# sdbds/ACE-Step-1.5-for-windows

Hardware: AMD Instinct MI355X
Metric: songs/sec (30 s audio @ 27 DiT steps, CFG 7 + APG, batch 8 in total, DiT + VAE decode) (higher is better)
Workload: dtype bf16; 1 GPU; acestep-5Hz base DiT (24L/2048d, 1.575B params, random init) + Oobleck decoder, 30 s audio (T=750), 27 steps, CFG 7 (2x8 sequences/forward on rank 0), L=769, 8 songs per request over 1 GPU(s); infer_steps=27, batch_per_gpu=8, batch_rank0=8, global_batch=8, parallelism=dp1, tiny=False, sampler_chains_per_gpu=1, batch_dependent_bits=True

## Files before the change

### ace-step-1.5-for-windows_amd/csrc/conv.hip

```cpp
#include <stdio.h>
#include <stdlib.h>

#include "common.h"


namespace ace355 {

namespace {

__device__ __forceinline__ int lds_off(int row, int slot) { return row * 128 + ((slot ^ ((row >> 1) & 7)) << 4); }

__device__ unsigned long long g_conv_probe[8];

typedef unsigned int u32x4 __attribute__((ext_vector_type(4)));
__device__ __forceinline__ u32x4 ld_u32x4(const void* p) {
    return *reinterpret_cast<const __attribute__((address_space(1))) u32x4*>(reinterpret_cast<uintptr_t>(p));
}

__device__ __forceinline__ void conv_glds16_v(const void* vptr, unsigned lds_addr) {
    unsigned keep;
    asm volatile("s_mov_b32 %0, m0\n\ts_mov_b32 m0, %2\n\ts_nop 0\n\tglobal_load_lds_dwordx4 %1, off\n\ts_mov_b32 m0, %0"
                 : "=&s"(keep)
                 : "v"(vptr), "s"(lds_addr)
                 : "memory");
}

constexpr int HALO_MAX = 64;

__device__ __forceinline__ void conv_glds16(unsigned voff, const void* sbase, unsigned lds_addr) {
    unsigned keep;
    asm volatile("s_mov_b32 %0, m0\n\ts_mov_b32 m0, %3\n\ts_nop 0\n\tglobal_load_lds_dwordx4 %1, %2\n\ts_mov_b32 m0, %0"
                 : "=&s"(keep)
                 : "v"(voff), "s"(sbase), "s"(lds_addr)
                 : "memory");
}

__device__ __forceinline__ bf16x8 frag_kperm(const char* base, int row, int q, int h) {
    const uint2 lo = *reinterpret_cast<const uint2*>(base + lds_off(row, 2 * q) + 8 * h);
    const uint2 hi = *reinterpret_cast<const uint2*>(base + lds_off(row, 2 * q + 1) + 8 * h);
    return as_bf16x8(make_uint4(lo.x, lo.y, hi.x, hi.y));
}

template <int BN, int TM, int WS = 0>
__global__ __launch_bounds__(TM * 2, TM / 64) void conv_kernel(ConvArgs a) {
    static_assert(TM == 128 || (TM == 256 && BN == 128), "tile shapes");
    static_assert(WS == 0 || (TM == 256 && BN == 128), "the 32 x 128 wave shape belongs to the fused 8-wave form");
    constexpr int NTHR = TM * 2;
    constexpr int WIN_MAX = TM + HALO_MAX;
    constexpr int MT = WS ? 1 : ((BN == 128) ? 2 : 1);
    constexpr int NT = WS ? 4 : ((BN == 128) ? 2 : 1);
    constexpr int WCH = BN * 8 / NTHR;
    constexpr int FUSE_LDS = (BN == 128 && TM == 128) ? (BN * 128 + 2048) : (WS ? 2048 : 0);
    __shared__ __attribute__((aligned(16))) char smem[WIN_MAX * 128 + 2 * BN * 128 + FUSE_LDS];
    char* As = smem;
    char* Wbase = smem + WIN_MAX * 128;

    const int tid = threadIdx.x, lane = tid & 63, wave = tid >> 6;
    const int lq = lane & 31, half = lane >> 5;
    const int wm = WS ? wave : ((BN == 128) ? (wave >> 1) : wave);
    const int wn = WS ? 0 : ((BN == 128) ? (wave & 1) : 0);
    int bx = blockIdx.x, by = blockIdx.y;
    if (a.ras_tn > 1) {
        const int L = blockIdx.x, tn = a.ras_tn, full = (a.ras_tm >> 3) << 3;
        if (L < full * tn) {
            const int q = L >> 3;
            by = q % tn;
            bx = (q / tn) * 8 + (L & 7);
        } else {
            const int l2 = L - full * tn;
            by = l2 % tn;
            bx = full + l2 / tn;
        }
    }
    const int m0 = bx * TM, n0 = by * BN, b = blockIdx.z;
    const int Cin = a.Cin, taps = a.taps, dil = a.dil;
    const int win_rows = TM + (taps - 1) * dil;
    const int x_row0 = m0 - a.center * dil;
    const bf16_t* xb = a.x + (long)b * a.x_batch_stride;
    const long wrow = (long)taps * Cin;

    f32x16 acc[MT][NT];
#pragma unroll
    for (int i = 0; i < MT; ++i)
#pragma unroll
        for (int j = 0; j < NT; ++j)
#pragma unroll
            for (int r = 0; r < 16; ++r) acc[i][j][r] = 0.f;

    const int sslot = tid & 7;
    constexpr int NWV = NTHR / 64;
    static_assert(WCH * NWV * 8 == BN, "pieces split evenly over the waves");
    unsigned w_voff[WCH];
    int wst[WCH];
#pragma unroll
    for (int i = 0; i < WCH; ++i) {
        const int prow = 8 * (wave + NWV * i) + (lane >> 3);
        const int ls = (lane & 7) ^ ((prow >> 1) & 7);
        w_voff[i] = (unsigned)(((long)min(n0 + prow, a.N - 1) * wrow + ls * 8) * 2);
        wst[i] = lds_off((tid >> 3) + (NTHR / 8) * i, sslot);
    }
    const unsigned wlds0 = (unsigned)(uintptr_t)Wbase + (unsigned)__builtin_amdgcn_readfirstlane(wave) * 1024u;
    auto w_piece = [&](int i, int tap, int ci0, int buf) {
        const bf16_t* sb = a.w + (long)tap * Cin + ci0;
        const unsigned lb = (unsigned)__builtin_amdgcn_readfirstlane((int)(wlds0 + (unsigned)buf * (BN * 128)));
        conv_glds16(w_voff[i], sb, lb + (unsigned)i * (NWV * 1024));
    };
    auto w_issue = [&](int tap, int ci0, int buf) {
#pragma unroll
        for (int i = 0; i < WCH; ++i) w_piece(i, tap, ci0, buf);
    };
    auto w2_piece = [&](int i, int c2, unsigned lbase) {
        const int prow = 8 * (wave + NWV * i) + (lane >> 3);
        const int ls = (lane & 7) ^ ((prow >> 1) & 7);
        conv_glds16((unsigned)((prow * 128 + ls * 8) * 2), a.w2 + c2 * 64, (unsigned)__builtin_amdgcn_readfirstlane((int)lbase) + (unsigned)i * (NWV * 1024));
    };

    constexpr int WLD = (WIN_MAX * 8 + NTHR - 1) / NTHR;
    constexpr bool PREFETCH = true;
    constexpr bool PARPRE = (TM == 128);
    u32x4 wv[WLD];
    const bool snake = a.alpha != nullptr;
    const int wrow_t = tid >> 3;
    const unsigned x_voff = (unsigned)((wrow_t * Cin + sslot * 8) * 2);
    const long xw_f0 = (long)x_row0 * Cin + a.x_shift;
    const long xw_end = a.x_valid ? a.x_valid : (long)a.L_in * Cin;
    const long xw_fb = max(xw_f0, 0L);
    const int xw_neg = (int)((xw_f0 - xw_fb) * 2);
    const uintptr_t xw_bp = reinterpret_cast<uintptr_t>(xb + xw_fb);
    const unsigned xw_lo32 = (unsigned)__builtin_amdgcn_readfirstlane((int)(unsigned)xw_bp);
    const unsigned xw_hi32 = (unsigned)__builtin_amdgcn_readfirstlane((int)(unsigned)(xw_bp >> 32));
    const unsigned xw_nrec = (unsigned)__builtin_amdgcn_readfirstlane((int)max(0L, min((xw_end - xw_fb) * 2, 0x7fffffffL)));
    const __amdgpu_buffer_rsrc_t x_rsrc =
        __builtin_amdgcn_make_buffer_rsrc(reinterpret_cast<void*>(((uintptr_t)xw_hi32 << 32) | xw_lo32), (short)0, (int)xw_nrec, 0x00020000);
    auto win_load = [&](int ci0) {
#pragma unroll
        for (int i = 0; i < WLD; ++i) {
            const int uoff = xw_neg + (i * (NTHR / 8) * Cin + ci0) * 2;
            const auto v = __builtin_amdgcn_raw_buffer_load_b128(x_rsrc, (int)x_voff + min(uoff, 0), max(uoff, 0), 0);
            wv[i] = __builtin_bit_cast(u32x4, v);
        }
    };
    u32x4 spa[2], spb[2];
    auto par_load = [&](int ci0) {
        if (snake) {
#pragma unroll
            for (int q = 0; q < 2; ++q) {
                spa[q] = ld_u32x4(a.alpha + ci0 + sslot * 8 + 4 * q);
                spb[q] = ld_u32x4(a.beta + ci0 + sslot * 8 + 4 * q);
            }
        }
    };
    const int st0 = lds_off(tid >> 3, sslot);
    auto vec_rsrc = [&](const float* p, int n) {
        const uintptr_t u = reinterpret_cast<uintptr_t>(p);
        const unsigned lo = (unsigned)__builtin_amdgcn_readfirstlane((int)(unsigned)u), hi = (unsigned)__builtin_amdgcn_readfirstlane((int)(unsigned)(u >> 32));
        return __builtin_amdgcn_make_buffer_rsrc(reinterpret_cast<void*>(((uintptr_t)hi << 32) | lo), (short)0, p ? n * 4 : 0, 0x00020000);
    };
    const __amdgpu_buffer_rsrc_t sa_rsrc = vec_rsrc(a.alpha, Cin), sb_rsrc = vec_rsrc(a.beta, Cin);
    auto snake_pair = [&](unsigned p, float a0, unsigned b0, float a1, unsigned b1) -> unsigned {
        const float x0 = bf_lo(p), x1 = bf_hi(p);
        const float s0 = __builtin_amdgcn_sinf(a0 * x0), s1 = __builtin_amdgcn_sinf(a1 * x1);
        return pack_bf2(x0 + __uint_as_float(b0) * s0 * s0, x1 + __uint_as_float(b1) * s1 * s1);
    };
    auto rev4 = [&](const u32x4& v, float (&o)[4]) {
#pragma unroll
        for (int e = 0; e < 4; ++e) o[e] = __uint_as_float(v[e]) * 0.15915494309189535f;
    };
    auto win_store = [&](int ci0) {
        if (snake) {
            if constexpr (PARPRE) {
                float ra[2][4];
                rev4(spa[0], ra[0]); rev4(spa[1], ra[1]);
#pragma unroll
                for (int i = 0; i < WLD; ++i)
#pragma unroll
                    for (int e2 = 0; e2 < 4; ++e2)
                        wv[i][e2] = snake_pair(wv[i][e2], ra[e2 >> 1][2 * (e2 & 1)], spb[e2 >> 1][2 * (e2 & 1)],
                                               ra[e2 >> 1][2 * (e2 & 1) + 1], spb[e2 >> 1][2 * (e2 & 1) + 1]);
            } else {
#pragma unroll
                for (int h = 0; h < 2; ++h) {
                    const u32x4 pa = __builtin_bit_cast(u32x4, __builtin_amdgcn_raw_buffer_load_b128(sa_rsrc, sslot * 32, (ci0 + 4 * h) * 4, 0));
                    const u32x4 pb = __builtin_bit_cast(u32x4, __builtin_amdgcn_raw_buffer_load_b128(sb_rsrc, sslot * 32, (ci0 + 4 * h) * 4, 0));
                    float ra[4];
                    rev4(pa, ra);
#pragma unroll
                    for (int i = 0; i < WLD; ++i)
#pragma unroll
                        for (int q = 0; q < 2; ++q)
                            wv[i][2 * h + q] = snake_pair(wv[i][2 * h + q], ra[2 * q], pb[2 * q], ra[2 * q + 1], pb[2 * q + 1]);
                    __builtin_amdgcn_sched_barrier(0);
                }
            }
        }
#pragma unroll
        for (int i = 0; i < WLD; ++i) {
            const int c = tid + i * NTHR;
            if (c < win_rows * 8) *reinterpret_cast<u32x4*>(As + st0 + i * (NTHR / 8) * 128) = wv[i];
        }
    };
    const bool probe = a.clk_probe && blockIdx.x == gridDim.x / 2 && blockIdx.y == 0 && blockIdx.z == 0 && __builtin_amdgcn_readfirstlane(wave) == 0;
    unsigned long long p_t0 = 0, p_w0 = 0, p_stage = 0, p_taps = 0, p_mark = 0;
    if (probe) p_t0 = clock64(), p_w0 = wall_clock64();
    constexpr bool FPIPE = (TM == 128);
    if (PREFETCH) { win_load(0); if (PARPRE) par_load(0); }
    for (int ci0 = 0; ci0 < Cin; ci0 += 64) {
        if (probe) p_mark = clock64();
        if (!PREFETCH) win_load(ci0);
        __syncthreads();
        if (PREFETCH) __builtin_amdgcn_s_waitcnt(0x0F70);
        w_issue(0, ci0, 0);
        win_store(ci0);
        asm volatile("s_waitcnt vmcnt(0)" ::: "memory");
        __syncthreads();
        if (PREFETCH && ci0 + 64 < Cin) { win_load(ci0 + 64); if (PARPRE) par_load(ci0 + 64); }
        if (probe) { const unsigned long long t = clock64(); p_stage += t - p_mark; p_mark = t; }

#pragma unroll 1
        for (int tap = 0; tap < taps; ++tap) {
            const bool more = (tap + 1) < taps;
            if (more) w_issue(tap + 1, ci0, (tap + 1) & 1);
            if constexpr (FUSE_LDS != 0) {
                if (a.w2 && ci0 + 64 >= Cin) {
                    constexpr int PT_OFF = (WS ? 2 : 3) * BN * 128;
                    if constexpr (WS == 0) {
                        const unsigned w2b = (unsigned)(uintptr_t)(Wbase + 2 * BN * 128) + (unsigned)__builtin_amdgcn_readfirstlane(wave) * 1024u;
                        if (tap >= 1 && tap <= WCH) w2_piece(tap - 1, 0, w2b);
                    }
                    if (tap == 5 && __builtin_amdgcn_readfirstlane(wave) < 2) {
                        const float* src = (wave == 0) ? (lane < 32 ? (a.bias ? a.bias : a.alpha2) : a.alpha2)
                                                       : (lane < 32 ? a.beta2 : (a.bias2 ? a.bias2 : a.beta2));
                        conv_glds16_v(src + 4 * (lane & 31), (unsigned)(uintptr_t)(Wbase + PT_OFF) + (unsigned)__builtin_amdgcn_readfirstlane(wave) * 1024u);
                    }
                    if (!more) {
                        const unsigned ring = wlds0 + (unsigned)((tap + 1) & 1) * (BN * 128);
#pragma unroll
                        for (int i = 0; i < WCH; ++i) w2_piece(i, WS ? 0 : 1, ring);
                    }
                }
            }
            const char* Ws = Wbase + (tap & 1) * (BN * 128);
            const int arow = wm * (MT * 32) + tap * dil + lq;
            if constexpr (FPIPE) {
                bf16x8 fa[2][MT], fw[2][NT];
                auto frag = [&](int kk, int sl) {
#pragma unroll
                    for (int i = 0; i < MT; ++i)
                        fa[sl][i] = as_bf16x8(*reinterpret_cast<const uint4*>(As + lds_off(arow + i * 32, kk * 2 + half)));
#pragma unroll
                    for (int j = 0; j < NT; ++j)
                        fw[sl][j] = as_bf16x8(*reinterpret_cast<const uint4*>(Ws + lds_off(wn * (NT * 32) + j * 32 + lq, kk * 2 + half)));
                };
                frag(0, 0);
#pragma unroll
                for (int kk = 0; kk < 4; ++kk) {
                    if (kk < 3) frag(kk + 1, (kk + 1) & 1);
                    __builtin_amdgcn_sched_barrier(0);
#pragma unroll
                    for (int i = 0; i < MT; ++i)
#pragma unroll
                        for (int j = 0; j < NT; ++j) acc[i][j] = mfma32(fw[kk & 1][j], fa[kk & 1][i], acc[i][j]);
                    __builtin_amdgcn_sched_barrier(0);
                }
            } else {
#pragma unroll
                for (int kk = 0; kk < 4; ++kk) {
                    bf16x8 fa[MT], fw[NT];
#pragma unroll
                    for (int i = 0; i < MT; ++i)
                        fa[i] = as_bf16x8(*reinterpret_cast<const uint4*>(As + lds_off(arow + i * 32, kk * 2 + half)));
#pragma unroll
                    for (int j = 0; j < NT; ++j)
                        fw[j] = as_bf16x8(*reinterpret_cast<const uint4*>(Ws + lds_off(wn * (NT * 32) + j * 32 + lq, kk * 2 + half)));
#pragma unroll
                    for (int i = 0; i < MT; ++i)
#pragma unroll
                        for (int j = 0; j < NT; ++j) acc[i][j] = mfma32(fw[j], fa[i], acc[i][j]);
                }
            }
            if (more) {
                asm volatile("s_waitcnt vmcnt(0)" ::: "memory");
                __syncthreads();
            }
        }
        if (probe) p_taps += clock64() - p_mark;
    }
    const bool full = (m0 + TM <= a.M) && (n0 + BN <= a.N) &&
                      ((long)m0 * a.N + n0 + a.y_shift >= 0) && ((long)(m0 + TM - 1) * a.N + n0 + BN - 1 + a.y_shift < a.y_valid);
    const bool wide = BN == 128 && a.out_mode == 0 && full && a.wide_ok;
    const int mw0 = m0 + wm * (MT * 32), nw0 = n0 + wn * (NT * 32);
    const int row_l = lane >> 2, c4 = lane & 3;
    u32x4 bl[NT], bh[NT];
    u32x4 rv[2][MT * 2];
    const bool has_res = (TM == 128 || WS == 1) && a.res != nullptr;
    auto res_load = [&](int j, u32x4 (&r)[MT * 2]) {
        const long rcol = (long)b * a.res_batch_stride + nw0 + j * 32 + c4 * 8 + a.y_shift;
#pragma unroll
        for (int t = 0; t < MT * 2; ++t) r[t] = ld_u32x4(a.res + rcol + (long)(mw0 + t * 16 + row_l) * a.N);
    };
    auto epi_pre = [&](const float* eb) {
#pragma unroll
        for (int j = 0; j < NT; ++j) {
            bl[j] = u32x4{0u, 0u, 0u, 0u};
            bh[j] = u32x4{0u, 0u, 0u, 0u};
        }
        if (eb && WS == 0) {
#pragma unroll
            for (int j = 0; j < NT; ++j) {
                bl[j] = ld_u32x4(eb + nw0 + j * 32 + c4 * 8);
                bh[j] = ld_u32x4(eb + nw0 + j * 32 + c4 * 8 + 4);
            }
        }
        if (has_res) res_load(0, rv[0]);
    };
    bool epi_pre_done = false;
    const float* epi_bias = a.bias;
    bool bias_in_lds = false;
    if constexpr (WS == 1) {
        if (a.w2) {
            epi_bias = a.bias2;
            bias_in_lds = a.bias2 != nullptr;
            const float b7s = a.bias ? 1.f : 0.f;
            const char* W2c0 = Wbase + (taps & 1) * (BN * 128);
            const char* W2c1 = Wbase + ((taps + 1) & 1) * (BN * 128);
            const char* Pt = Wbase + 2 * BN * 128;
            __syncthreads();
            {
                const unsigned ring = wlds0 + (unsigned)(taps & 1 ? 0 : 1) * (BN * 128);
#pragma unroll
                for (int i = 0; i < WCH; ++i) w2_piece(i, 1, ring);
            }
            uint2 sp[NT][4];
#pragma unroll
            for (int j = 0; j < NT; ++j)
#pragma unroll
                for (int g = 0; g < 4; ++g) {
                    const int c = j * 32 + 8 * g + 4 * half;
                    const u32x4 b4 = *reinterpret_cast<const u32x4*>(Pt + c * 4);
                    const u32x4 e4 = *reinterpret_cast<const u32x4*>(Pt + 512 + c * 4);
                    const u32x4 i4 = *reinterpret_cast<const u32x4*>(Pt + 1024 + c * 4);
                    float t[4];
#pragma unroll
                    for (int e = 0; e < 4; ++e) {
                        const float v = acc[0][j][4 * g + e] + b7s * __uint_as_float(b4[e]);
                        const float sn = __sinf(__uint_as_float(e4[e]) * v);
                        t[e] = v + __uint_as_float(i4[e]) * sn * sn;
                    }
                    sp[j][g] = make_uint2(pack_bf2(t[0], t[1]), pack_bf2(t[2], t[3]));
                    __builtin_amdgcn_sched_barrier(0);
                }
#pragma unroll
            for (int j = 0; j < NT; ++j)
#pragma unroll
                for (int r = 0; r < 16; ++r) acc[0][j][r] = 0.f;
            asm volatile("s_waitcnt vmcnt(0)" ::: "memory");
            __syncthreads();
#pragma unroll
            for (int kg = 0; kg < 8; ++kg) {
                const char* Wp = (kg >> 2) ? W2c1 : W2c0;
                const uint2 s0 = sp[kg >> 1][2 * (kg & 1)], s1 = sp[kg >> 1][2 * (kg & 1) + 1];
                const bf16x8 fb = as_bf16x8(make_uint4(s0.x, s0.y, s1.x, s1.y));
                bf16x8 fw[NT];
#pragma unroll
                for (int j = 0; j < NT; ++j) fw[j] = frag_kperm(Wp, j * 32 + lq, kg & 3, half);
#pragma unroll
                for (int j = 0; j < NT; ++j) acc[0][j] = mfma32(fw[j], fb, acc[0][j]);
            }
        }
    }
    if constexpr (BN == 128 && TM == 128) {
        if (a.w2) {
            epi_bias = a.bias2;
            const float* b7p = a.bias ? a.bias : a.alpha2;
            const float b7s = a.bias ? 1.f : 0.f;
            __syncthreads();
            char* A2 = smem;
            const char* W2c0 = Wbase + 2 * BN * 128;
            const char* W2c1 = Wbase + (taps & 1) * (BN * 128);
            const char* Pt = Wbase + 3 * BN * 128;
#pragma unroll
            for (int j = 0; j < NT; ++j) {
                u32x4 b4[4], e4[4], i4[4];
#pragma unroll
                for (int g = 0; g < 4; ++g) {
                    const int c = n0 + wn * (NT * 32) + j * 32 + 8 * g + 4 * half;
                    b4[g] = *reinterpret_cast<const u32x4*>(Pt + c * 4);
                    e4[g] = *reinterpret_cast<const u32x4*>(Pt + 512 + c * 4);
                    i4[g] = *reinterpret_cast<const u32x4*>(Pt + 1024 + c * 4);
                }
#pragma unroll
                for (int i = 0; i < MT; ++i)
#pragma unroll
                    for (int g = 0; g < 4; ++g) {
                        float t[4];
#pragma unroll
                        for (int e = 0; e < 4; ++e) {
                            const float v = acc[i][j][4 * g + e] + b7s * __uint_as_float(b4[g][e]);
                            const float sn = __sinf(__uint_as_float(e4[g][e]) * v);
                            t[e] = v + __uint_as_float(i4[g][e]) * sn * sn;
                        }
                        const int row = wm * (MT * 32) + i * 32 + lq;
                        uint2 pk = make_uint2(pack_bf2(t[0], t[1]), pack_bf2(t[2], t[3]));
                        *reinterpret_cast<uint2*>(A2 + wn * 16384 + lds_off(row, j * 4 + g) + 8 * half) = pk;
                    }
            }
#pragma unroll
            for (int i = 0; i < MT; ++i)
#pragma unroll
                for (int j = 0; j < NT; ++j)
#pragma unroll
                    for (int r = 0; r < 16; ++r) acc[i][j][r] = 0.f;
            asm volatile("s_waitcnt vmcnt(0)" ::: "memory");
            __syncthreads();
            if (wide) { epi_pre(a.bias2); epi_pre_done = true; }
            {
                bf16x8 fa[2][MT], fw[2][NT];
                auto frag2 = [&](int k8, int sl) {
                    const char* Ap = A2 + (k8 >> 2) * 16384;
                    const char* Wp = (k8 >> 2) ? W2c1 : W2c0;
                    const int kk = k8 & 3;
#pragma unroll
                    for (int i = 0; i < MT; ++i) fa[sl][i] = frag_kperm(Ap, wm * (MT * 32) + i * 32 + lq, kk, half);
#pragma unroll
                    for (int j = 0; j < NT; ++j) fw[sl][j] = frag_kperm(Wp, wn * (NT * 32) + j * 32 + lq, kk, half);
                };
                frag2(0, 0);
#pragma unroll
                for (int k8 = 0; k8 < 8; ++k8) {
                    if (k8 < 7) frag2(k8 + 1, (k8 + 1) & 1);
                    __builtin_amdgcn_sched_barrier(0);
#pragma unroll
                    for (int i = 0; i < MT; ++i)
#pragma unroll
                        for (int j = 0; j < NT; ++j) acc[i][j] = mfma32(fw[k8 & 1][j], fa[k8 & 1][i], acc[i][j]);
                    __builtin_amdgcn_sched_barrier(0);
                }
            }
        }
    }
    const unsigned long long p_e0 = probe ? clock64() : 0ull;
    auto probe_done = [&]() {
        if (!probe) return;
        __builtin_amdgcn_s_waitcnt(0x0F70);
        const unsigned long long t = clock64();
        g_conv_probe[0] = t - p_t0, g_conv_probe[1] = p_stage, g_conv_probe[2] = p_taps, g_conv_probe[3] = t - p_e0;
        g_conv_probe[4] = wall_clock64() - p_w0, g_conv_probe[5] = (unsigned long long)(Cin / 64);
    };

    if (wide) {
        if (!epi_pre_done) epi_pre(epi_bias);
        __syncthreads();
        char* stg = smem + wave * (MT * 32 * 128);
#pragma unroll
        for (int j = 0; j < NT; ++j) {
#pragma unroll
            for (int i = 0; i < MT; ++i)
#pragma unroll
                for (int g = 0; g < 4; ++g) {
                    float4 v;
                    v.x = acc[i][j][4 * g + 0]; v.y = acc[i][j][4 * g + 1]; v.z = acc[i][j][4 * g + 2]; v.w = acc[i][j][4 * g + 3];
                    const int row = i * 32 + lq, slot = 2 * g + half;
                    *reinterpret_cast<float4*>(stg + row * 128 + ((slot ^ (row & 7)) << 4)) = v;
                }
            if (has_res && j + 1 < NT) res_load(j + 1, rv[(j + 1) & 1]);
            u32x4 oa[2], ob[2];
            if (a.osnake_a) {
#pragma unroll
                for (int q = 0; q < 2; ++q) {
                    oa[q] = ld_u32x4(a.osnake_a + nw0 + j * 32 + c4 * 8 + 4 * q);
                    ob[q] = ld_u32x4(a.osnake_b + nw0 + j * 32 + c4 * 8 + 4 * q);
                }
            }
            const long col = (long)b * a.y_batch_stride + nw0 + j * 32 + c4 * 8 + a.y_shift;
            if constexpr (WS == 1) {
                if (bias_in_lds) {
                    const char* pb = Wbase + 2 * BN * 128 + 1536 + (nw0 + j * 32 + c4 * 8) * 4;
                    bl[j] = *reinterpret_cast<const u32x4*>(pb);
                    bh[j] = *reinterpret_cast<const u32x4*>(pb + 16);
                } else if (epi_bias) {
                    bl[j] = ld_u32x4(epi_bias + nw0 + j * 32 + c4 * 8);
                    bh[j] = ld_u32x4(epi_bias + nw0 + j * 32 + c4 * 8 + 4);
                }
            }
            const float bias[8] = {__uint_as_float(bl[j][0]), __uint_as_float(bl[j][1]), __uint_as_float(bl[j][2]), __uint_as_float(bl[j][3]),
                                   __uint_as_float(bh[j][0]), __uint_as_float(bh[j][1]), __uint_as_float(bh[j][2]), __uint_as_float(bh[j][3])};
#pragma unroll
            for (int t = 0; t < MT * 2; ++t) {
                const int row = t * 16 + row_l;
                const float4 lo = *reinterpret_cast<const float4*>(stg + row * 128 + (((2 * c4) ^ (row & 7)) << 4));
                const float4 hi = *reinterpret_cast<const float4*>(stg + row * 128 + (((2 * c4 + 1) ^ (row & 7)) << 4));
                float v[8] = {lo.x + bias[0], lo.y + bias[1], lo.z + bias[2], lo.w + bias[3],
                              hi.x + bias[4], hi.y + bias[5], hi.z + bias[6], hi.w + bias[7]};
                if (has_res) {
                    const u32x4 r = rv[j & 1][t];
#pragma unroll
                    for (int e2 = 0; e2 < 4; ++e2) { v[2 * e2] += bf_lo(r[e2]); v[2 * e2 + 1] += bf_hi(r[e2]); }
                }
                if (a.osnake_a) {
#pragma unroll
                    for (int e = 0; e < 8; ++e) {
                        const float sn = __sinf(__uint_as_float(oa[e >> 2][e & 3]) * v[e]);
                        v[e] = v[e] + __uint_as_float(ob[e >> 2][e & 3]) * sn * sn;
                    }
                }
                u32x4 pk = {pack_bf2(v[0], v[1]), pack_bf2(v[2], v[3]), pack_bf2(v[4], v[5]), pack_bf2(v[6], v[7])};
                *reinterpret_cast<u32x4*>(reinterpret_cast<bf16_t*>(a.y) + col + (long)(mw0 + row) * a.N) = pk;
            }
        }
        probe_done();
        return;
    }
#pragma unroll
    for (int i = 0; i < MT; ++i) {
        const int m = mw0 + i * 32 + lq;
        if (m >= a.M) continue;
#pragma unroll
        for (int j = 0; j < NT; ++j)
#pragma unroll
            for (int r = 0; r < 16; ++r) {
                const int n = nw0 + j * 32 + 8 * (r >> 2) + 4 * half + (r & 3);
                if (n >= a.N) continue;
                float v = acc[i][j][r] + (epi_bias ? epi_bias[n] : 0.f);
                if (a.out_mode == 0) {
                    const long flat = (long)m * a.N + n + a.y_shift;
                    if (flat < 0 || flat >= a.y_valid) continue;
                    if (a.res) v += bf2f(a.res[(long)b * a.res_batch_stride + flat]);
                    if (a.osnake_a) {
                        const float sn = __sinf(a.osnake_a[n] * v);
                        v = v + a.osnake_b[n] * sn * sn;
                    }
                    reinterpret_cast<bf16_t*>(a.y)[(long)b * a.y_batch_stride + flat] = f2bf(v);
                } else {
                    if (n < a.n_real) {
                        if (a.ncl_ld == 0) reinterpret_cast<float*>(a.y)[(long)b * a.y_batch_stride + (long)n * a.M + m] = v;
                        else if (m >= a.ncl_m_lo && m < a.ncl_m_hi)
                            reinterpret_cast<float*>(a.y)[(long)b * a.y_batch_stride + (long)n * a.ncl_ld + a.ncl_off + (m - a.ncl_m_lo)] = v;
                    }
                }
            }
    }
}

__global__ void ncl_to_nlc_kernel(const float* __restrict__ z, bf16_t* __restrict__ out, int C, int T, long total) {
    const long i = (long)blockIdx.x * blockDim.x + threadIdx.x;
    if (i >= total) return;
    const int c = (int)(i % C);
    const long bt = i / C;
    const int t = (int)(bt % T);
    const long b = bt / T;
    out[i] = f2bf(z[(b * C + c) * T + t]);
}

}

int launch_conv(const ConvArgs& a, hipStream_t s) {
    ACE_CHECK(a.Cin % 64 == 0, "conv: Cin must be a multiple of 64");
    ACE_CHECK(a.taps >= 1 && (a.taps - 1) * a.dil <= HALO_MAX && a.dil >= 1, "conv: window too large");
    ACE_CHECK(a.B > 0 && a.M > 0 && a.N > 0, "conv: empty problem");
    ACE_CHECK((long)a.N * a.taps * a.Cin * 2 < (1L << 32) && (reinterpret_cast<uintptr_t>(a.w) & 15) == 0,
              "conv: the weight tensor must be 16-byte aligned and smaller than 4 GB (32-bit DMA offsets)");
    ACE_CHECK(a.x_valid ? (a.x_shift % 8 == 0 && a.x_valid % 8 == 0) : a.x_shift == 0, "conv: x_shift / x_valid must be multiples of 8 (and x_shift needs x_valid)");
    ACE_CHECK(!a.w2 || (a.Cin == 128 && a.N == 128 && a.taps == 7 && !a.x_valid && a.out_mode == 0 && a.alpha2 && a.beta2 &&
                        (reinterpret_cast<uintptr_t>(a.alpha2) & 15) == 0 && (reinterpret_cast<uintptr_t>(a.beta2) & 15) == 0 &&
                        (reinterpret_cast<uintptr_t>(a.bias) & 15) == 0 && (reinterpret_cast<uintptr_t>(a.w2) & 15) == 0),
              "conv: the fused k = 1 stage needs Cin = N = 128, a plain conv and 16-byte aligned vectors");
    ACE_CHECK(!a.osnake_a == !a.osnake_b && (!a.osnake_a || a.out_mode == 0), "conv: the producer-side Snake needs both parameter vectors and the bf16 output");
    ConvArgs aw = a;
    {
        auto al16 = [](const void* p) { return (reinterpret_cast<uintptr_t>(p) & 15) == 0; };
        aw.wide_ok = a.out_mode == 0 && al16(a.y) && al16(a.res) && al16(a.bias) && al16(a.bias2) && al16(a.osnake_a) && al16(a.osnake_b) &&
                     (a.N % 8) == 0 && (a.y_shift % 8) == 0 &&
                     (a.y_batch_stride % 8) == 0 && (a.res_batch_stride % 8) == 0;
    }
    static int tm_env = -1, clk_env = -1, ras_env = -1;
    if (ras_env < 0) {
        const char* e = getenv("ACE355_CONV_RAS");
        ras_env = e ? atoi(e) : 1;
    }
    if (clk_env < 0) {
        const char* e = getenv("ACE355_CONV_CLK");
        clk_env = e ? atoi(e) : 0;
    }
    aw.clk_probe = clk_env;
    if (tm_env < 0) {
        const char* e = getenv("ACE355_CONV_TM");
        tm_env = e ? atoi(e) : 0;
    }
    if (a.N >= 128 || a.N % 128 == 0) {
        const long wgs128 = (long)((a.M + 127) / 128) * ((a.N + 127) / 128) * a.B;
        const bool tall_k = a.Cin >= 128 && a.taps >= 3 && wgs128 >= 1400;
        const bool tall_t = a.taps == 2 && a.Cin >= 128 && !a.alpha && !a.x_valid && wgs128 >= 1500;
        const bool tall = !a.w2 && !a.res && (tm_env ? tm_env == 256 : (tall_k || tall_t));
        const int tm_rows = tall ? 256 : 128;
        dim3 grid((a.M + tm_rows - 1) / tm_rows, (a.N + 127) / 128, a.B);
        aw.ras_tm = aw.ras_tn = 0;
        if (ras_env && grid.y > 1 && (long)grid.x * grid.y < (1L << 31)) {
            aw.ras_tm = (int)grid.x, aw.ras_tn = (int)grid.y;
            grid = dim3(grid.x * grid.y, 1, a.B);
        }
        static int f8_env = -2;
        if (f8_env == -2) {
            const char* e = getenv("ACE355_CONV_F8");
            f8_env = e ? atoi(e) : -1;
        }
        const bool f8 = a.w2 && (f8_env >= 0 ? f8_env != 0 : wgs128 >= 1400);
        if (f8) {
            dim3 g8((a.M + 255) / 256, 1, a.B);
            aw.ras_tm = aw.ras_tn = 0;
            hipLaunchKernelGGL((conv_kernel<128, 256, 1>), g8, dim3(512), 0, s, aw);
        } else
        if (tall) hipLaunchKernelGGL((conv_kernel<128, 256>), grid, dim3(512), 0, s, aw);
        else hipLaunchKernelGGL((conv_kernel<128, 128>), grid, dim3(256), 0, s, aw);
    } else {
        aw.ras_tm = aw.ras_tn = 0;
        dim3 grid((a.M + 127) / 128, (a.N + 31) / 32, a.B);
        hipLaunchKernelGGL((conv_kernel<32, 128>), grid, dim3(256), 0, s, aw);
    }
    ACE_LAUNCH_CHECK();
    if (aw.clk_probe) {
        ACE_HIP(hipStreamSynchronize(s));
        unsigned long long h[8];
        ACE_HIP(hipMemcpyFromSymbol(h, HIP_SYMBOL(g_conv_probe), sizeof(h)));
        fprintf(stderr, "[conv clk] Cin=%d N=%d taps=%d dil=%d M=%d: total %llu cyc = stage %llu + taps %llu + epilogue %llu (+%llu other), wall %.2f us, %llu chunks\n",
                a.Cin, a.N, a.taps, a.dil, a.M, h[0], h[1], h[2], h[3], h[0] - h[1] - h[2] - h[3], h[4] / 100.0, h[5]);
    }
    return 0;
}

int launch_ncl_to_nlc(const float* z, bf16_t* out, int B, int C, int T, hipStream_t s) {
    const long total = (long)B * C * T;
    hipLaunchKernelGGL(ncl_to_nlc_kernel, dim3((unsigned)((total + 255) / 256)), dim3(256), 0, s, z, out, C, T, total);
    ACE_LAUNCH_CHECK();
    return 0;
}

}
```

### ace-step-1.5-for-windows_amd/csrc/vae.hip

```cpp
#include <math.h>
#include <string.h>

#include <algorithm>
#include <map>
#include <string>
#include <vector>

#include "encoder.h"

using namespace ace355;

namespace {

struct ConvW {
    bf16_t* w = nullptr;
    float* bias = nullptr;
    int N = 0, taps = 0, Cin = 0;
};
struct SnakeP {
    float* ea = nullptr;
    float* ib = nullptr;
};
struct ResUnitW {
    SnakeP s1, s2;
// ... 395 lines not shown
    h->finalized = false;
    return ACE355_OK;
}

int ace355_vae_finalize(ace355_vae* h) {
    ACE_CHECK(h, "vae_finalize: null handle");
    const ace355_vae_config& c = h->cfg;
    const int nb = c.num_blocks;
    int cm[ACE355_MAX_BLOCKS + 1];
    cm[0] = 1;
    for (int i = 0; i < nb; ++i) cm[i + 1] = c.channel_multiples[i];
    int rc;
    const int C0 = c.decoder_channels * cm[nb];
    if ((rc = build_conv(h, "decoder.conv1", C0, c.decoder_input_channels, 7, true, &h->conv1))) return rc;
    h->blocks.assign(nb, BlockW());
    for (int i = 0; i < nb; ++i) {
        BlockW& B = h->blocks[i];
        B.cin = c.decoder_channels * cm[nb - i];
        B.cout = c.decoder_channels * cm[nb - i - 1];
        B.stride = c.upsampling_ratios[i];
        B.pad = (B.stride + 1) / 2;
        ACE_CHECK(B.cin % 64 == 0 && B.cout % 64 == 0, "vae_finalize: block channels must be multiples of 64");
        const std::string p = "decoder.block." + std::to_string(i);
        if ((rc = build_snake(h, p + ".snake1", B.cin, &B.s1))) return rc;
        if ((rc = build_convt(h, p + ".conv_t1", B.cin, B.cout, B.stride, &B.ct))) return rc;
        const int dils[3] = {1, 3, 9};
        for (int j = 0; j < 3; ++j) {
            ResUnitW& R = B.ru[j];
            R.dil = dils[j];
            const std::string r = p + ".res_unit" + std::to_string(j + 1);
            if ((rc = build_snake(h, r + ".snake1", B.cout, &R.s1))) return rc;
            if ((rc = build_conv(h, r + ".conv1", B.cout, B.cout, 7, true, &R.c1))) return rc;
            if ((rc = build_snake(h, r + ".snake2", B.cout, &R.s2))) return rc;
            if ((rc = build_conv(h, r + ".conv2", B.cout, B.cout, 1, true, &R.c2))) return rc;
        }
    }
    if ((rc = build_snake(h, "decoder.snake1", c.decoder_channels, &h->s_out))) return rc;
    if ((rc = build_conv(h, "decoder.conv2", c.audio_channels, c.decoder_channels, 7, false, &h->conv2))) return rc;
    h->has_encoder = false;
    for (auto& kv : h->raw) if (kv.first.rfind("encoder.", 0) == 0) { h->has_encoder = true; break; }
    if (h->has_encoder) {
        const int EH = 2 * c.decoder_input_channels;
        ACE_CHECK(EH % 64 == 0, "vae_finalize: encoder width must be a multiple of 64");
        if ((rc = build_conv_im2col(h, "encoder.conv1", EH, c.audio_channels, 7, &h->e_conv1))) return rc;
        h->e_blocks.assign(nb, EncBlockW());
        for (int i = 0; i < nb; ++i) {
            EncBlockW& B = h->e_blocks[i];
            B.cin = EH * cm[i];
            B.cout = EH * cm[i + 1];
            B.stride = c.upsampling_ratios[nb - 1 - i];
            B.pad = (B.stride + 1) / 2;
            ACE_CHECK(B.cin % 64 == 0 && B.cout % 64 == 0, "vae_finalize: encoder block channels must be multiples of 64");
            const std::string p = "encoder.block." + std::to_string(i);
            const int dils[3] = {1, 3, 9};
            for (int j = 0; j < 3; ++j)
                if ((rc = build_res_unit(h, p + ".res_unit" + std::to_string(j + 1), B.cin, dils[j], &B.ru[j]))) return rc;
            if ((rc = build_snake_tiled(h, p + ".snake1", B.cin, B.stride, &B.s1))) return rc;
            if ((rc = build_conv_strided(h, p + ".conv1", B.cout, B.cin, B.stride, &B.cd))) return rc;
        }
        if ((rc = build_snake(h, "encoder.snake1", EH * cm[nb], &h->e_s_out))) return rc;
        if ((rc = build_conv(h, "encoder.conv2", EH, EH * cm[nb], 3, true, &h->e_conv2))) return rc;
    }
    ACE_HIP(hipDeviceSynchronize());
    for (auto& kv : h->raw) {
        const std::string& k = kv.first;
        const bool keep = k.size() > 5 && k.compare(k.size() - 5, 5, ".bias") == 0;
        if (!keep && kv.second.p) { hipFree(kv.second.p); kv.second.p = nullptr; }
    }
    if (!h->scratch) ACE_HIP(hipMalloc((void**)&h->scratch, 1024));
    h->finalized = true;
    return ACE355_OK;
}

int ace355_vae_hop(const ace355_vae* h) { return h ? h->hop : 0; }

static int episnake_on() {
    static int on = -1;
    if (on < 0) {
        const char* e = getenv("ACE355_VAE_EPISNAKE");
        on = e ? atoi(e) : 1;
    }
    return on;
}
static bool unit_fused(int C) {
    static int fuse = -1;
    if (fuse < 0) {
        const char* e = getenv("ACE355_CONV_FUSE_RU");
        fuse = e ? atoi(e) : 1;
    }
    return fuse && C == 128;
}

static void stage_push(std::vector<ace355_vae_stage_info>& v, int kind, int block, int unit, int channels, int flags, int src, int res,
                       int dil, long rows) {
    ace355_vae_stage_info si;
    si.kind = kind; si.block = block; si.unit = unit; si.channels = channels; si.flags = flags; si.src = src; si.res = res;
    si.dilation = dil; si.rows = rows;
    v.push_back(si);
}
static void stage_push_unit(std::vector<ace355_vae_stage_info>& v, int block, int unit, int C, int dil, long rows, bool epi, bool out_snake) {
    const int in = (int)v.size() - 1;
    const int osn = out_snake ? ACE355_VAE_FLAG_OUT_SNAKE : 0;
    if (unit_fused(C)) {
        stage_push(v, ACE355_VAE_STAGE_UNIT, block, unit, C, ACE355_VAE_FLAG_FUSED | ACE355_VAE_FLAG_IN_SNAKE | osn, in, in, dil, rows);
        return;
    }
    stage_push(v, ACE355_VAE_STAGE_UNIT_K7, block, unit, C, ACE355_VAE_FLAG_IN_SNAKE | (epi ? ACE355_VAE_FLAG_OUT_SNAKE : 0), in, -1, dil, rows);
    stage_push(v, ACE355_VAE_STAGE_UNIT_K1, block, unit, C, (epi ? 0 : ACE355_VAE_FLAG_IN_SNAKE) | osn, in + 1, in, 1, rows);
}
static int stage_list(const ace355_vae* h, int enc, long T, std::vector<ace355_vae_stage_info>& v) {
    v.clear();
    const ace355_vae_config& c = h->cfg;
    if (!enc) {
        const bool epi = episnake_on() != 0 && !h->blocks.empty();
        stage_push(v, ACE355_VAE_STAGE_INPUT, -1, -1, c.decoder_input_channels, 0, -1, -1, 1, T);
        stage_push(v, ACE355_VAE_STAGE_CONV_IN, -1, -1, h->conv1.N, epi ? ACE355_VAE_FLAG_OUT_SNAKE : 0, 0, -1, 1, T);
        long L = T;
        for (size_t bi = 0; bi < h->blocks.size(); ++bi) {
            const BlockW& Bk = h->blocks[bi];
            L = (L - 1) * Bk.stride - 2 * Bk.pad + 2 * Bk.stride;
            stage_push(v, ACE355_VAE_STAGE_CONVT, (int)bi, -1, Bk.cout, epi ? 0 : ACE355_VAE_FLAG_IN_SNAKE, (int)v.size() - 1, -1, 1, L);
            for (int j = 0; j < 3; ++j) stage_push_unit(v, (int)bi, j, Bk.cout, Bk.ru[j].dil, L, epi, epi && j == 2);
        }
        return 0;
    }
    const bool epi = episnake_on() != 0;
    const int EH = 2 * c.decoder_input_channels;
    stage_push(v, ACE355_VAE_STAGE_INPUT, -1, -1, 64, 0, -1, -1, 1, T);
    stage_push(v, ACE355_VAE_STAGE_CONV_IN, -1, -1, EH, 0, 0, -1, 1, T);
    long L = T;
    for (size_t bi = 0; bi < h->e_blocks.size(); ++bi) {
        const EncBlockW& Bk = h->e_blocks[bi];
        for (int j = 0; j < 3; ++j) stage_push_unit(v, (int)bi, j, Bk.cin, Bk.ru[j].dil, L, epi, epi && j == 2);
        L = (L + 2 * Bk.pad - 2 * Bk.stride) / Bk.stride + 1;
        ACE_CHECK(L > 0, "vae stages: audio shorter than one latent frame");
        stage_push(v, ACE355_VAE_STAGE_DOWN, (int)bi, -1, Bk.cout,
                   (epi ? 0 : ACE355_VAE_FLAG_IN_SNAKE) | (epi && bi + 1 == h->e_blocks.size() ? ACE355_VAE_FLAG_OUT_SNAKE : 0), (int)v.size() - 1,
                   -1, 1, L);
    }
    stage_push(v, ACE355_VAE_STAGE_HEAD, -1, -1, EH,
               ACE355_VAE_FLAG_F32_NCL | ((!epi || h->e_blocks.empty()) ? ACE355_VAE_FLAG_IN_SNAKE : 0), (int)v.size() - 1, -1, 1, L);
    return 0;
}
static int tap_stage(ace355_vae* h, int enc, int kind, const void* p, int B, hipStream_t s) {
    if (h->tap_stages.empty()) return 0;
    const int k = h->tap_next++;
    ACE_CHECK(k < (int)h->tap_stages.size() && h->tap_stages[k].kind == kind, "vae tap: the stage list and the launch sequence disagree");
    auto it = h->taps[enc].find(k);
    if (it == h->taps[enc].end()) return 0;
    const ace355_vae_stage_info& si = h->tap_stages[k];
    const size_t bytes = (size_t)B * si.rows * si.channels * ((si.flags & ACE355_VAE_FLAG_F32_NCL) ? 4 : 2);
    ACE_CHECK(bytes <= it->second.second, "vae tap: the destination is smaller than the stage");
    ACE_HIP(hipMemcpyAsync(it->second.first, p, bytes, hipMemcpyDeviceToDevice, s));
    return 0;
}
static int tap_begin(ace355_vae* h, int enc, long T, bool single_window) {
    h->tap_stages.clear();
    h->tap_next = 0;
    if (h->taps[enc].empty()) return 0;
    if (!single_window) {
        set_error("vae tap: the call splits into several windows under the activation budget; a tap needs one whole-sequence window");
        return ACE355_ERR_STATE;
    }
    int rc = stage_list(h, enc, T, h->tap_stages);
    if (rc) { h->tap_stages.clear(); return rc; }
    ACE_CHECK(h->taps[enc].rbegin()->first < (int)h->tap_stages.size(), "vae tap: no such stage");
    return 0;
}
static int tap_end(ace355_vae* h) {
    const bool ok = h->tap_stages.empty() || h->tap_next == (int)h->tap_stages.size();
    h->tap_stages.clear();
    ACE_CHECK(ok, "vae tap: the stage list and the launch sequence disagree");
    return 0;
}

static int run_res_unit(ace355_vae* h, const ResUnitW& R, bf16_t*& state, bf16_t*& tmp, int B, long L, int C, hipStream_t s,
                        int enc, const SnakeP* out_snake = nullptr) {
    if (unit_fused(C)) {
        ConvArgs f{};
        f.x = state; f.x_batch_stride = L * C; f.L_in = (int)L; f.Cin = C;
        f.w = R.c1.w; f.bias = R.c1.bias; f.alpha = R.s1.ea; f.beta = R.s1.ib;
        f.w2 = R.c2.w; f.bias2 = R.c2.bias; f.alpha2 = R.s2.ea; f.beta2 = R.s2.ib;
        f.res = state; f.res_batch_stride = L * C;
        f.y = tmp; f.y_batch_stride = L * C;
        f.B = B; f.M = (int)L; f.N = C; f.taps = 7; f.dil = R.dil; f.center = 3;
        f.y_shift = 0; f.y_valid = L * C; f.out_mode = 0;
        if (out_snake) f.osnake_a = out_snake->ea, f.osnake_b = out_snake->ib;
        const int rcf = run_conv(h, f, s);
        if (rcf) return rcf;
        std::swap(state, tmp);
        return tap_stage(h, enc, ACE355_VAE_STAGE_UNIT, state, B, s);
    }
    ConvArgs a{};
    a.x = state; a.x_batch_stride = L * C; a.L_in = (int)L; a.Cin = C;
    a.w = R.c1.w; a.bias = R.c1.bias; a.alpha = R.s1.ea; a.beta = R.s1.ib;
    a.y = tmp; a.y_batch_stride = L * C;
    a.B = B; a.M = (int)L; a.N = C; a.taps = 7; a.dil = R.dil; a.center = 3;
    a.y_shift = 0; a.y_valid = L * C; a.out_mode = 0;
    const bool epi = episnake_on() != 0;
    if (epi) a.osnake_a = R.s2.ea, a.osnake_b = R.s2.ib;
    int rc = run_conv(h, a, s);
    if (rc) return rc;
    if ((rc = tap_stage(h, enc, ACE355_VAE_STAGE_UNIT_K7, tmp, B, s))) return rc;
    a = ConvArgs{};
    a.x = tmp; a.x_batch_stride = L * C; a.L_in = (int)L; a.Cin = C;
    a.w = R.c2.w; a.bias = R.c2.bias;
    if (!epi) a.alpha = R.s2.ea, a.beta = R.s2.ib;
    if (out_snake) a.osnake_a = out_snake->ea, a.osnake_b = out_snake->ib;
    a.res = state; a.res_batch_stride = L * C;
    a.y = state; a.y_batch_stride = L * C;
    a.B = B; a.M = (int)L; a.N = C; a.taps = 1; a.dil = 1; a.center = 0;
    a.y_shift = 0; a.y_valid = L * C; a.out_mode = 0;
    if ((rc = run_conv(h, a, s))) return rc;
    return tap_stage(h, enc, ACE355_VAE_STAGE_UNIT_K1, state, B, s);
}

static size_t decode_elems(const ace355_vae* h, long frames) {
    size_t need = (size_t)frames * h->conv1.N;
    long L = frames;
    for (const BlockW& Bk : h->blocks) {
        L = (L - 1) * Bk.stride - 2 * Bk.pad + 2 * Bk.stride;
        need = std::max(need, (size_t)L * Bk.cout);
    }
    return need;
}
static size_t decode_bytes(const ace355_vae* h, int nb, long frames) { return 3 * (decode_elems(h, frames) * (size_t)nb * 2 + 256); }

static int decode_receptive_frames(const ace355_vae* h) {
    double rf = 3.0, rate = 1.0;
    for (const BlockW& Bk : h->blocks) {
        rf += 1.0 / rate;
        rate *= Bk.stride;
        rf += 3.0 * (1 + 3 + 9) / rate;
    }
    rf += 3.0 / rate;
    return (int)ceil(rf);
}

static int decode_window(ace355_vae* h, int b0, int nb, int T, int ws, int we, int cs, int ce, float* wav_out_dev, hipStream_t s) {
    const ace355_vae_config& c = h->cfg;
    const int Tw = we - ws;
    bf16_t *cur = h->buf[0], *nxt = h->buf[1], *tmp = h->buf[2];
    long L = Tw;
    int rc;
    ConvArgs a{};
    a.x = h->zin + ((size_t)b0 * T + ws) * c.decoder_input_channels; a.x_batch_stride = (long)T * c.decoder_input_channels; a.L_in = Tw;
    a.Cin = c.decoder_input_channels;
    a.w = h->conv1.w; a.bias = h->conv1.bias;
    a.y = cur; a.y_batch_stride = (long)Tw * h->conv1.N;
    a.B = nb; a.M = Tw; a.N = h->conv1.N; a.taps = 7; a.dil = 1; a.center = 3;
    a.y_shift = 0; a.y_valid = (long)Tw * h->conv1.N; a.out_mode = 0;
    const bool epi = episnake_on() != 0 && !h->blocks.empty();
    if (epi) a.osnake_a = h->blocks[0].s1.ea, a.osnake_b = h->blocks[0].s1.ib;
    if ((rc = run_conv(h, a, s))) return rc;
    if ((rc = tap_stage(h, 0, ACE355_VAE_STAGE_CONV_IN, cur, nb, s))) return rc;

    for (size_t bi = 0; bi < h->blocks.size(); ++bi) {
        const BlockW& Bk = h->blocks[bi];
        const SnakeP* next_snake = !epi ? nullptr : (bi + 1 < h->blocks.size() ? &h->blocks[bi + 1].s1 : &h->s_out);
        const long Lout = (L - 1) * Bk.stride - 2 * Bk.pad + 2 * Bk.stride;
        a = ConvArgs{};
// ... 304 lines not shown
```

Before: 17.50 songs/s.

## Extend fused residual-unit conv kernel to 256-channel decoder stages

Generalizes the fused k=7 conv + Snake + k=1 conv residual-unit kernel from 128 channels to 256 channels by adding a 256x256 tile, 8-wave variant. The k=1 weight chunks are streamed through the double-buffered LDS ring with extra barriers, and the parameter and bias vectors are laid out by BN. Decoder residual units at C=256 now use this single kernel instead of separate conv launches, which removes an intermediate activation round-trip through global memory. The trade-offs are a larger LDS footprint and lower occupancy (launch bounds of 2), plus extra synchronization inside the epilogue.

```diff
diff --git a/ace-step-1.5-for-windows_amd/csrc/conv.hip b/ace-step-1.5-for-windows_amd/csrc/conv.hip
--- a/ace-step-1.5-for-windows_amd/csrc/conv.hip
+++ b/ace-step-1.5-for-windows_amd/csrc/conv.hip
@@ -42,15 +42,15 @@
 }
 
 template <int BN, int TM, int WS = 0>
-__global__ __launch_bounds__(TM * 2, TM / 64) void conv_kernel(ConvArgs a) {
-    static_assert(TM == 128 || (TM == 256 && BN == 128), "tile shapes");
-    static_assert(WS == 0 || (TM == 256 && BN == 128), "the 32 x 128 wave shape belongs to the fused 8-wave form");
+__global__ __launch_bounds__(TM * 2, (WS && BN == 256) ? 2 : TM / 64) void conv_kernel(ConvArgs a) {
+    static_assert(TM == 128 || (TM == 256 && (BN == 128 || (BN == 256 && WS == 1))), "tile shapes");
+    static_assert(WS == 0 || (TM == 256 && BN >= 128), "the 32 x BN wave shape belongs to the fused 8-wave forms");
     constexpr int NTHR = TM * 2;
     constexpr int WIN_MAX = TM + HALO_MAX;
     constexpr int MT = WS ? 1 : ((BN == 128) ? 2 : 1);
-    constexpr int NT = WS ? 4 : ((BN == 128) ? 2 : 1);
+    constexpr int NT = WS ? BN / 32 : ((BN == 128) ? 2 : 1);
     constexpr int WCH = BN * 8 / NTHR;
-    constexpr int FUSE_LDS = (BN == 128 && TM == 128) ? (BN * 128 + 2048) : (WS ? 2048 : 0);
+    constexpr int FUSE_LDS = (BN == 128 && TM == 128) ? (BN * 128 + 2048) : (WS ? BN * 16 : 0);
     __shared__ __attribute__((aligned(16))) char smem[WIN_MAX * 128 + 2 * BN * 128 + FUSE_LDS];
     char* As = smem;
     char* Wbase = smem + WIN_MAX * 128;
@@ -112,7 +112,7 @@
     auto w2_piece = [&](int i, int c2, unsigned lbase) {
         const int prow = 8 * (wave + NWV * i) + (lane >> 3);
         const int ls = (lane & 7) ^ ((prow >> 1) & 7);
-        conv_glds16((unsigned)((prow * 128 + ls * 8) * 2), a.w2 + c2 * 64, (unsigned)__builtin_amdgcn_readfirstlane((int)lbase) + (unsigned)i * (NWV * 1024));
+        conv_glds16((unsigned)((prow * BN + ls * 8) * 2), a.w2 + c2 * 64, (unsigned)__builtin_amdgcn_readfirstlane((int)lbase) + (unsigned)i * (NWV * 1024));
     };
 
     constexpr int WLD = (WIN_MAX * 8 + NTHR - 1) / NTHR;
@@ -227,10 +227,11 @@
                         const unsigned w2b = (unsigned)(uintptr_t)(Wbase + 2 * BN * 128) + (unsigned)__builtin_amdgcn_readfirstlane(wave) * 1024u;
                         if (tap >= 1 && tap <= WCH) w2_piece(tap - 1, 0, w2b);
                     }
-                    if (tap == 5 && __builtin_amdgcn_readfirstlane(wave) < 2) {
-                        const float* src = (wave == 0) ? (lane < 32 ? (a.bias ? a.bias : a.alpha2) : a.alpha2)
-                                                       : (lane < 32 ? a.beta2 : (a.bias2 ? a.bias2 : a.beta2));
-                        conv_glds16_v(src + 4 * (lane & 31), (unsigned)(uintptr_t)(Wbase + PT_OFF) + (unsigned)__builtin_amdgcn_readfirstlane(wave) * 1024u);
+                    if (tap == 5 && __builtin_amdgcn_readfirstlane(wave) < BN / 64) {
+                        constexpr int LPV = BN / 4;
+                        const int vec = (wave * 64 + lane) / LPV;
+                        const float* src = vec == 0 ? (a.bias ? a.bias : a.alpha2) : vec == 1 ? a.alpha2 : vec == 2 ? a.beta2 : (a.bias2 ? a.bias2 : a.beta2);
+                        conv_glds16_v(src + 4 * ((wave * 64 + lane) % LPV), (unsigned)(uintptr_t)(Wbase + PT_OFF) + (unsigned)__builtin_amdgcn_readfirstlane(wave) * 1024u);
                     }
                     if (!more) {
                         const unsigned ring = wlds0 + (unsigned)((tap + 1) & 1) * (BN * 128);
@@ -287,7 +288,7 @@
     }
     const bool full = (m0 + TM <= a.M) && (n0 + BN <= a.N) &&
                       ((long)m0 * a.N + n0 + a.y_shift >= 0) && ((long)(m0 + TM - 1) * a.N + n0 + BN - 1 + a.y_shift < a.y_valid);
-    const bool wide = BN == 128 && a.out_mode == 0 && full && a.wide_ok;
+    const bool wide = BN >= 128 && a.out_mode == 0 && full && a.wide_ok;
     const int mw0 = m0 + wm * (MT * 32), nw0 = n0 + wn * (NT * 32);
     const int row_l = lane >> 2, c4 = lane & 3;
     u32x4 bl[NT], bh[NT];
@@ -321,8 +322,7 @@
             epi_bias = a.bias2;
             bias_in_lds = a.bias2 != nullptr;
             const float b7s = a.bias ? 1.f : 0.f;
-            const char* W2c0 = Wbase + (taps & 1) * (BN * 128);
-            const char* W2c1 = Wbase + ((taps + 1) & 1) * (BN * 128);
+            constexpr int NC2 = BN / 64;
             const char* Pt = Wbase + 2 * BN * 128;
             __syncthreads();
             {
@@ -337,8 +337,8 @@
                 for (int g = 0; g < 4; ++g) {
                     const int c = j * 32 + 8 * g + 4 * half;
                     const u32x4 b4 = *reinterpret_cast<const u32x4*>(Pt + c * 4);
-                    const u32x4 e4 = *reinterpret_cast<const u32x4*>(Pt + 512 + c * 4);
-                    const u32x4 i4 = *reinterpret_cast<const u32x4*>(Pt + 1024 + c * 4);
+                    const u32x4 e4 = *reinterpret_cast<const u32x4*>(Pt + BN * 4 + c * 4);
+                    const u32x4 i4 = *reinterpret_cast<const u32x4*>(Pt + BN * 8 + c * 4);
                     float t[4];
 #pragma unroll
                     for (int e = 0; e < 4; ++e) {
@@ -356,15 +356,30 @@
             asm volatile("s_waitcnt vmcnt(0)" ::: "memory");
             __syncthreads();
 #pragma unroll
-            for (int kg = 0; kg < 8; ++kg) {
-                const char* Wp = (kg >> 2) ? W2c1 : W2c0;
-                const uint2 s0 = sp[kg >> 1][2 * (kg & 1)], s1 = sp[kg >> 1][2 * (kg & 1) + 1];
-                const bf16x8 fb = as_bf16x8(make_uint4(s0.x, s0.y, s1.x, s1.y));
-                bf16x8 fw[NT];
-#pragma unroll
-                for (int j = 0; j < NT; ++j) fw[j] = frag_kperm(Wp, j * 32 + lq, kg & 3, half);
-#pragma unroll
-                for (int j = 0; j < NT; ++j) acc[0][j] = mfma32(fw[j], fb, acc[0][j]);
+            for (int c2 = 0; c2 < NC2; ++c2) {
+                const char* Wp = Wbase + ((taps + c2) & 1) * (BN * 128);
+#pragma unroll
+                for (int k4 = 0; k4 < 4; ++k4) {
+                    const int kg = 4 * c2 + k4;
+                    const uint2 s0 = sp[kg >> 1][2 * (kg & 1)], s1 = sp[kg >> 1][2 * (kg & 1) + 1];
+                    const bf16x8 fb = as_bf16x8(make_uint4(s0.x, s0.y, s1.x, s1.y));
+                    bf16x8 fw[NT];
+#pragma unroll
+                    for (int j = 0; j < NT; ++j) fw[j] = frag_kperm(Wp, j * 32 + lq, k4, half);
+#pragma unroll
+                    for (int j = 0; j < NT; ++j) acc[0][j] = mfma32(fw[j], fb, acc[0][j]);
+                }
+                if constexpr (NC2 > 2) {
+                    if (c2 + 1 < NC2) {
+                        asm volatile("s_waitcnt vmcnt(0)" ::: "memory");
+                        __syncthreads();
+                        if (c2 + 2 < NC2) {
+                            const unsigned ring = wlds0 + (unsigned)((taps + c2) & 1) * (BN * 128);
+#pragma unroll
+                            for (int i = 0; i < WCH; ++i) w2_piece(i, c2 + 2, ring);
+                        }
+                    }
+                }
             }
         }
     }
@@ -474,7 +489,7 @@
             const long col = (long)b * a.y_batch_stride + nw0 + j * 32 + c4 * 8 + a.y_shift;
             if constexpr (WS == 1) {
                 if (bias_in_lds) {
-                    const char* pb = Wbase + 2 * BN * 128 + 1536 + (nw0 + j * 32 + c4 * 8) * 4;
+                    const char* pb = Wbase + 2 * BN * 128 + BN * 12 + (nw0 + j * 32 + c4 * 8) * 4;
                     bl[j] = *reinterpret_cast<const u32x4*>(pb);
                     bh[j] = *reinterpret_cast<const u32x4*>(pb + 16);
                 } else if (epi_bias) {
@@ -560,10 +575,11 @@
     ACE_CHECK((long)a.N * a.taps * a.Cin * 2 < (1L << 32) && (reinterpret_cast<uintptr_t>(a.w) & 15) == 0,
               "conv: the weight tensor must be 16-byte aligned and smaller than 4 GB (32-bit DMA offsets)");
     ACE_CHECK(a.x_valid ? (a.x_shift % 8 == 0 && a.x_valid % 8 == 0) : a.x_shift == 0, "conv: x_shift / x_valid must be multiples of 8 (and x_shift needs x_valid)");
-    ACE_CHECK(!a.w2 || (a.Cin == 128 && a.N == 128 && a.taps == 7 && !a.x_valid && a.out_mode == 0 && a.alpha2 && a.beta2 &&
+    ACE_CHECK(!a.w2 || ((a.Cin == 128 || a.Cin == 256) && a.N == a.Cin && a.taps == 7 && !a.x_valid && a.out_mode == 0 && a.alpha2 && a.beta2 &&
                         (reinterpret_cast<uintptr_t>(a.alpha2) & 15) == 0 && (reinterpret_cast<uintptr_t>(a.beta2) & 15) == 0 &&
-                        (reinterpret_cast<uintptr_t>(a.bias) & 15) == 0 && (reinterpret_cast<uintptr_t>(a.w2) & 15) == 0),
-              "conv: the fused k = 1 stage needs Cin = N = 128, a plain conv and 16-byte aligned vectors");
+                        (reinterpret_cast<uintptr_t>(a.bias) & 15) == 0 && (reinterpret_cast<uintptr_t>(a.bias2) & 15) == 0 &&
+                        (reinterpret_cast<uintptr_t>(a.w2) & 15) == 0),
+              "conv: the fused k = 1 stage needs Cin = N = 128 or 256, a plain conv and 16-byte aligned vectors");
     ACE_CHECK(!a.osnake_a == !a.osnake_b && (!a.osnake_a || a.out_mode == 0), "conv: the producer-side Snake needs both parameter vectors and the bf16 output");
     ConvArgs aw = a;
     {
@@ -604,6 +620,11 @@
             f8_env = e ? atoi(e) : -1;
         }
         const bool f8 = a.w2 && (f8_env >= 0 ? f8_env != 0 : wgs128 >= 1400);
+        if (a.w2 && a.N == 256) {
+            dim3 g8((a.M + 255) / 256, 1, a.B);
+            aw.ras_tm = aw.ras_tn = 0;
+            hipLaunchKernelGGL((conv_kernel<256, 256, 1>), g8, dim3(512), 0, s, aw);
+        } else
         if (f8) {
             dim3 g8((a.M + 255) / 256, 1, a.B);
             aw.ras_tm = aw.ras_tn = 0;
diff --git a/ace-step-1.5-for-windows_amd/csrc/vae.hip b/ace-step-1.5-for-windows_amd/csrc/vae.hip
--- a/ace-step-1.5-for-windows_amd/csrc/vae.hip
+++ b/ace-step-1.5-for-windows_amd/csrc/vae.hip
@@ -501,13 +501,13 @@
     }
     return on;
 }
-static bool unit_fused(int C) {
+static bool unit_fused(int C, int enc) {
     static int fuse = -1;
     if (fuse < 0) {
         const char* e = getenv("ACE355_CONV_FUSE_RU");
         fuse = e ? atoi(e) : 1;
     }
-    return fuse && C == 128;
+    return fuse == 128 ? C == 128 : (fuse && (C == 128 || (C == 256 && !enc)));
 }
 
 static void stage_push(std::vector<ace355_vae_stage_info>& v, int kind, int block, int unit, int channels, int flags, int src, int res,
@@ -517,10 +517,10 @@
     si.dilation = dil; si.rows = rows;
     v.push_back(si);
 }
-static void stage_push_unit(std::vector<ace355_vae_stage_info>& v, int block, int unit, int C, int dil, long rows, bool epi, bool out_snake) {
+static void stage_push_unit(std::vector<ace355_vae_stage_info>& v, int enc, int block, int unit, int C, int dil, long rows, bool epi, bool out_snake) {
     const int in = (int)v.size() - 1;
     const int osn = out_snake ? ACE355_VAE_FLAG_OUT_SNAKE : 0;
-    if (unit_fused(C)) {
+    if (unit_fused(C, enc)) {
         stage_push(v, ACE355_VAE_STAGE_UNIT, block, unit, C, ACE355_VAE_FLAG_FUSED | ACE355_VAE_FLAG_IN_SNAKE | osn, in, in, dil, rows);
         return;
     }
@@ -539,7 +539,7 @@
             const BlockW& Bk = h->blocks[bi];
             L = (L - 1) * Bk.stride - 2 * Bk.pad + 2 * Bk.stride;
             stage_push(v, ACE355_VAE_STAGE_CONVT, (int)bi, -1, Bk.cout, epi ? 0 : ACE355_VAE_FLAG_IN_SNAKE, (int)v.size() - 1, -1, 1, L);
-            for (int j = 0; j < 3; ++j) stage_push_unit(v, (int)bi, j, Bk.cout, Bk.ru[j].dil, L, epi, epi && j == 2);
+            for (int j = 0; j < 3; ++j) stage_push_unit(v, 0, (int)bi, j, Bk.cout, Bk.ru[j].dil, L, epi, epi && j == 2);
         }
         return 0;
     }
@@ -550,7 +550,7 @@
     long L = T;
     for (size_t bi = 0; bi < h->e_blocks.size(); ++bi) {
         const EncBlockW& Bk = h->e_blocks[bi];
-        for (int j = 0; j < 3; ++j) stage_push_unit(v, (int)bi, j, Bk.cin, Bk.ru[j].dil, L, epi, epi && j == 2);
+        for (int j = 0; j < 3; ++j) stage_push_unit(v, 1, (int)bi, j, Bk.cin, Bk.ru[j].dil, L, epi, epi && j == 2);
         L = (L + 2 * Bk.pad - 2 * Bk.stride) / Bk.stride + 1;
         ACE_CHECK(L > 0, "vae stages: audio shorter than one latent frame");
         stage_push(v, ACE355_VAE_STAGE_DOWN, (int)bi, -1, Bk.cout,
@@ -595,7 +595,7 @@
 
 static int run_res_unit(ace355_vae* h, const ResUnitW& R, bf16_t*& state, bf16_t*& tmp, int B, long L, int C, hipStream_t s,
                         int enc, const SnakeP* out_snake = nullptr) {
-    if (unit_fused(C)) {
+    if (unit_fused(C, enc)) {
         ConvArgs f{};
         f.x = state; f.x_batch_stride = L * C; f.L_in = (int)L; f.Cin = C;
         f.w = R.c1.w; f.bias = R.c1.bias; f.alpha = R.s1.ea; f.beta = R.s1.ib;
```

Result: no change. 17.56 songs/s, median of 6 (+0.3%).
